# CompVis/behavior-driven-video-synthesis

Hardware: AMD Instinct MI355X
Metric: frames/sec VUnet 256x256 bs=16 fwd+bwd (higher is better)
Workload: dtype f32 (operands scaled by a power of two and split into 2 fp16 terms, 3 partial products on fp16 MFMA, fp32 accumulate; weight gradients and uncovered layers: 3 bf16 terms / 6 products, fp32-input MFMA, fp32 VALU); 1 GPU; Human3.6m shape_and_pose_net VunetAlter 256x256 per-GPU bs=16 fwd+bwd, VGG19 perceptual + KL loss, fused Adam, dropout 0.05, regressor side loop off, seeded-synthetic VGG19 weights, rasterised synthetic stickmen; global_batch=16, parallelism=dp1, conv_precision=h2, hip_streams=4, hip_graph=True, graph_settle_steps=7, rccl_world_size=1, dp_backend=none

## Files before the change

### behavior_driven_video_synthesis_amd/csrc/planes.hip

```cpp
#include "common.h"
#include "split_h2.h"

namespace {

constexpr int P2_AMAX0 = 16, P2_NSLOT = 64;

__device__ __forceinline__ void p2_unpack8(const uint4& h, const uint4& l, float inv, float* v) {
  const uint32_t hs[4] = {h.x, h.y, h.z, h.w}, ls[4] = {l.x, l.y, l.z, l.w};
#pragma unroll
  for (int j = 0; j < 4; ++j) {
    const h2_f16x2 a = __builtin_bit_cast(h2_f16x2, hs[j]), b = __builtin_bit_cast(h2_f16x2, ls[j]);
    v[2 * j] = ((float)a[0] + (float)b[0] * (1.f / 2048.f)) * inv;
    v[2 * j + 1] = ((float)a[1] + (float)b[1] * (1.f / 2048.f)) * inv;
  }
}
__device__ __forceinline__ void p2_pack8(const float* v, float s, uint4& h, uint4& l) {
  h2_split2(v[0] * s, v[1] * s, h.x, l.x);
  h2_split2(v[2] * s, v[3] * s, h.y, l.y);
  h2_split2(v[4] * s, v[5] * s, h.z, l.z);
  h2_split2(v[6] * s, v[7] * s, h.w, l.w);
}
__device__ __forceinline__ float block_sum4(float v, float* red) {
  v = wave_sum(v);
  __syncthreads();
  if ((threadIdx.x & 63) == 0) red[threadIdx.x >> 6] = v;
  __syncthreads();
  return red[0] + red[1] + red[2] + red[3];
}
__device__ __forceinline__ float meta_amax(const int* meta) {
  return wave_max(__int_as_float(meta[P2_AMAX0 + (threadIdx.x & (P2_NSLOT - 1))]));
}
__device__ __forceinline__ void publish_amax(int* meta, float vmax) {
  const float m = wave_max(vmax);
  if ((threadIdx.x & 63) == 0)
    atomicMax(reinterpret_cast<unsigned*>(meta) + P2_AMAX0 + ((blockIdx.x * 4u + (threadIdx.x >> 6)) & (P2_NSLOT - 1)), __float_as_uint(m));
}

__global__ __launch_bounds__(256) void p2_finish_sum_kernel(const float* partial, int nb, float* out, float scale) {
  __shared__ float red[4];
  float s = 0.f;
  for (int i = threadIdx.x; i < nb; i += 256) s += partial[i];
  const float t = block_sum4(s, red);
  if (threadIdx.x == 0) out[0] += scale * t;
}

__global__ __launch_bounds__(256) void p2_l1_partial_kernel(const uint4* __restrict__ t, const int* __restrict__ tmeta,
                                                            const uint4* __restrict__ p, const int* __restrict__ pmeta,
                                                            float* __restrict__ partial, size_t plane) {
  __shared__ float red[4];
  const float it = h2_pow2(-tmeta[0]), ip = h2_pow2(-pmeta[0]);
  float s = 0.f;
  for (size_t i = (size_t)blockIdx.x * 256 + threadIdx.x; i < plane; i += (size_t)gridDim.x * 256) {
    float a[8], b[8];
    p2_unpack8(t[i], t[plane + i], it, a);
    p2_unpack8(p[i], p[plane + i], ip, b);
    s += ((fabsf(a[0] - b[0]) + fabsf(a[1] - b[1])) + (fabsf(a[2] - b[2]) + fabsf(a[3] - b[3]))) +
         ((fabsf(a[4] - b[4]) + fabsf(a[5] - b[5])) + (fabsf(a[6] - b[6]) + fabsf(a[7] - b[7])));
  }
  const float tot = block_sum4(s, red);
  if (threadIdx.x == 0) partial[blockIdx.x] = tot;
}

template <bool L1>
__global__ __launch_bounds__(256) void p2_pool_fwd_kernel(const uint4* __restrict__ t, const int* __restrict__ tmeta,
                                                          const uint4* __restrict__ p, const int* __restrict__ pmeta,
                                                          float* __restrict__ partial, uint4* __restrict__ y, int* __restrict__ ymeta,
                                                          int NCB, int H, int W) {
  __shared__ float red[4];
  const int Ho = H >> 1, Wo = W >> 1, Wp = W + 2, Wpo = Wo + 2;
  const size_t plane = (size_t)NCB * (H + 2) * Wp, plane_o = (size_t)NCB * (Ho + 2) * Wpo, total = (size_t)NCB * Ho * Wo;
  const float ip = h2_pow2(-pmeta[0]);
  const float it = L1 ? h2_pow2(-tmeta[0]) : 0.f;
  if (blockIdx.x == 0 && threadIdx.x < 64) {
    if (threadIdx.x == 0) ymeta[0] = pmeta[0];
    ymeta[P2_AMAX0 + threadIdx.x] = pmeta[P2_AMAX0 + threadIdx.x];
  }
  float s = 0.f;
  for (size_t o = (size_t)blockIdx.x * 256 + threadIdx.x; o < total; o += (size_t)gridDim.x * 256) {
    const int xo = (int)(o % Wo);
    size_t r = o / Wo;
    const int yo = (int)(r % Ho);
    const size_t ncb = r / Ho;
    const size_t i0 = (ncb * (H + 2) + (2 * yo + 1)) * Wp + (2 * xo + 1);
    const size_t off[4] = {i0, i0 + 1, i0 + Wp, i0 + Wp + 1};
    uint32_t hs[4][4], ls[4][4];
    float v[4][8];
#pragma unroll
    for (int e = 0; e < 4; ++e) {
      const uint4 h = p[off[e]], l = p[plane + off[e]];
      hs[e][0] = h.x; hs[e][1] = h.y; hs[e][2] = h.z; hs[e][3] = h.w;
      ls[e][0] = l.x; ls[e][1] = l.y; ls[e][2] = l.z; ls[e][3] = l.w;
      p2_unpack8(h, l, ip, v[e]);
    }
    if (L1) {
#pragma unroll
      for (int e = 0; e < 4; ++e) {
        float a[8];
        p2_unpack8(t[off[e]], t[plane + off[e]], it, a);
#pragma unroll
        for (int j = 0; j < 8; ++j) s += fabsf(a[j] - v[e][j]);
      }
    }
    uint32_t oh[4] = {0, 0, 0, 0}, ol[4] = {0, 0, 0, 0};
#pragma unroll
    for (int j = 0; j < 8; ++j) {
      const float m = fmaxf(fmaxf(v[0][j], v[1][j]), fmaxf(v[2][j], v[3][j]));
      const int k = v[0][j] == m ? 0 : (v[1][j] == m ? 1 : (v[2][j] == m ? 2 : 3));
      const uint32_t hsel = k == 0 ? hs[0][j >> 1] : (k == 1 ? hs[1][j >> 1] : (k == 2 ? hs[2][j >> 1] : hs[3][j >> 1]));
      const uint32_t lsel = k == 0 ? ls[0][j >> 1] : (k == 1 ? ls[1][j >> 1] : (k == 2 ? ls[2][j >> 1] : ls[3][j >> 1]));
      const uint32_t keep = (j & 1) ? 0xFFFF0000u : 0x0000FFFFu;
      oh[j >> 1] |= hsel & keep;
      ol[j >> 1] |= lsel & keep;
    }
    const size_t oo = (ncb * (Ho + 2) + (yo + 1)) * Wpo + (xo + 1);
    y[oo] = make_uint4(oh[0], oh[1], oh[2], oh[3]);
    y[plane_o + oo] = make_uint4(ol[0], ol[1], ol[2], ol[3]);
  }
  if (L1) {
    const float tot = block_sum4(s, red);
    if (threadIdx.x == 0) partial[blockIdx.x] = tot;
  }
}

__global__ __launch_bounds__(256) void p2_l1_bwd_kernel(const uint4* __restrict__ t, const int* __restrict__ tmeta,
                                                        const uint4* __restrict__ p, const int* __restrict__ pmeta,
                                                        const uint4* __restrict__ add, const int* __restrict__ addmeta,
                                                        uint4* __restrict__ g, int* __restrict__ gmeta, float gscale,
                                                        const float* __restrict__ gout, int NCB, int H, int W) {
  const float c = gscale * (gout ? gout[0] : 1.f);
  const float bound = (add ? meta_amax(addmeta) : 0.f) + fabsf(c);
  const int eg = h2_scale_exp(bound);
  const float sg = h2_pow2(eg);
  if (blockIdx.x == 0 && threadIdx.x == 0) gmeta[0] = eg;
  const float it = h2_pow2(-tmeta[0]), ip = h2_pow2(-pmeta[0]), ia = add ? h2_pow2(-addmeta[0]) : 0.f;
  const int Wp = W + 2;
  const size_t plane = (size_t)NCB * (H + 2) * Wp, total = (size_t)NCB * H * W;
  float vmax = 0.f;
  for (size_t o = (size_t)blockIdx.x * 256 + threadIdx.x; o < total; o += (size_t)gridDim.x * 256) {
    const int xw = (int)(o % W);
    size_t r = o / W;
    const int yh = (int)(r % H);
    const size_t i = ((r / H) * (H + 2) + (yh + 1)) * Wp + (xw + 1);
    float a[8], b[8], d[8];
    p2_unpack8(t[i], t[plane + i], it, a);
    p2_unpack8(p[i], p[plane + i], ip, b);
    if (add) p2_unpack8(add[i], add[plane + i], ia, d);
#pragma unroll
    for (int j = 0; j < 8; ++j) {
      const float df = b[j] - a[j];
      float v = (add ? d[j] : 0.f) + (df > 0.f ? c : (df < 0.f ? -c : 0.f));
      if (!(b[j] > 0.f)) v = 0.f;
      d[j] = v;
      vmax = fmaxf(vmax, fabsf(v));
    }
    uint4 h, l;
    p2_pack8(d, sg, h, l);
    g[i] = h;
    g[plane + i] = l;
  }
  publish_amax(gmeta, vmax);
}

template <bool L1>
__global__ __launch_bounds__(256) void p2_pool_bwd_kernel(const uint4* __restrict__ t, const int* __restrict__ tmeta,
                                                          const uint4* __restrict__ p, const int* __restrict__ pmeta,
                                                          const uint4* __restrict__ dy, const int* __restrict__ dymeta,
                                                          uint4* __restrict__ g, int* __restrict__ gmeta, float gscale,
                                                          const float* __restrict__ gout, int NCB, int H, int W) {
  const float c = L1 ? gscale * (gout ? gout[0] : 1.f) : 0.f;
  const float bound = meta_amax(dymeta) + fabsf(c);
  const int eg = h2_scale_exp(bound);
  const float sg = h2_pow2(eg);
  if (blockIdx.x == 0 && threadIdx.x == 0) gmeta[0] = eg;
  const float ip = h2_pow2(-pmeta[0]), idy = h2_pow2(-dymeta[0]);
  const float it = L1 ? h2_pow2(-tmeta[0]) : 0.f;
  const int Ho = H >> 1, Wo = W >> 1, Wp = W + 2, Wpo = Wo + 2;
  const size_t plane = (size_t)NCB * (H + 2) * Wp, plane_o = (size_t)NCB * (Ho + 2) * Wpo, total = (size_t)NCB * Ho * Wo;
  float vmax = 0.f;
  for (size_t o = (size_t)blockIdx.x * 256 + threadIdx.x; o < total; o += (size_t)gridDim.x * 256) {
    const int xo = (int)(o % Wo);
    size_t r = o / Wo;
    const int yo = (int)(r % Ho);
    const size_t ncb = r / Ho;
    const size_t i0 = (ncb * (H + 2) + (2 * yo + 1)) * Wp + (2 * xo + 1);
    const size_t off[4] = {i0, i0 + 1, i0 + Wp, i0 + Wp + 1};
    const size_t oo = (ncb * (Ho + 2) + (yo + 1)) * Wpo + (xo + 1);
    float v[4][8], gy[8];
#pragma unroll
    for (int e = 0; e < 4; ++e) p2_unpack8(p[off[e]], p[plane + off[e]], ip, v[e]);
    p2_unpack8(dy[oo], dy[plane_o + oo], idy, gy);
    float res[4][8];
#pragma unroll
    for (int j = 0; j < 8; ++j) {
      const float m = fmaxf(fmaxf(v[0][j], v[1][j]), fmaxf(v[2][j], v[3][j]));
      const int k = v[0][j] == m ? 0 : (v[1][j] == m ? 1 : (v[2][j] == m ? 2 : 3));
#pragma unroll
      for (int e = 0; e < 4; ++e) res[e][j] = k == e ? gy[j] : 0.f;
    }
#pragma unroll
    for (int e = 0; e < 4; ++e) {
      float a[8];
      if (L1) p2_unpack8(t[off[e]], t[plane + off[e]], it, a);
#pragma unroll
      for (int j = 0; j < 8; ++j) {
        float x = res[e][j];
        if (L1) {
          const float df = v[e][j] - a[j];
          x += df > 0.f ? c : (df < 0.f ? -c : 0.f);
        }
        if (!(v[e][j] > 0.f)) x = 0.f;
        res[e][j] = x;
        vmax = fmaxf(vmax, fabsf(x));
      }
      uint4 h, l;
      p2_pack8(res[e], sg, h, l);
      g[off[e]] = h;
      g[plane + off[e]] = l;
    }
  }
  publish_amax(gmeta, vmax);
}

inline unsigned grid_for(size_t n, unsigned cap) {
  size_t b = (n + 255) / 256;
  if (b > cap) b = cap;
  if (b < 1) b = 1;
  return (unsigned)b;
}

}

extern "C" int vunet_p2_l1_fwd(const void* t, const int32_t* tmeta, const void* p, const int32_t* pmeta, float* partial, float* out,
                               float weight, int32_t N, int32_t C, int32_t H, int32_t W, void* stream) {
  if (!t || !tmeta || !p || !pmeta || !partial || !out || C % 8 || N < 1) return VUNET_ERR_ARG;
  const size_t plane = (size_t)N * (C / 8) * (H + 2) * (W + 2);
  const unsigned nb = grid_for(plane, 1024);
  hipStream_t st = (hipStream_t)stream;
  VUNET_LAUNCH(p2_l1_partial_kernel, dim3(nb), dim3(256), 0, st, (const uint4*)t, (const int*)tmeta, (const uint4*)p, (const int*)pmeta,
               partial, plane);
  VUNET_LAUNCH(p2_finish_sum_kernel, dim3(1), dim3(256), 0, st, (const float*)partial, (int)nb, out,
               weight / ((float)N * C * H * W));
  return vunet_check_launch();
}

extern "C" int vunet_p2_pool_fwd(const void* t, const int32_t* tmeta, const void* p, const int32_t* pmeta, float* partial, float* out,
                                 float weight, void* y, int32_t* ymeta, int32_t N, int32_t C, int32_t H, int32_t W, void* stream) {
  if (!p || !pmeta || !y || !ymeta || C % 8 || N < 1 || (H & 1) || (W & 1)) return VUNET_ERR_ARG;
  if (t && (!tmeta || !partial || !out)) return VUNET_ERR_ARG;
  const int NCB = N * (C / 8);
  const size_t total = (size_t)NCB * (H / 2) * (W / 2);
  const unsigned nb = grid_for(total, 1024);
  hipStream_t st = (hipStream_t)stream;
  if (t) {
    VUNET_LAUNCH(p2_pool_fwd_kernel<true>, dim3(nb), dim3(256), 0, st, (const uint4*)t, (const int*)tmeta, (const uint4*)p,
                 (const int*)pmeta, partial, (uint4*)y, (int*)ymeta, NCB, (int)H, (int)W);
    VUNET_LAUNCH(p2_finish_sum_kernel, dim3(1), dim3(256), 0, st, (const float*)partial, (int)nb, out,
                 weight / ((float)N * C * H * W));
  } else {
    VUNET_LAUNCH(p2_pool_fwd_kernel<false>, dim3(nb), dim3(256), 0, st, (const uint4*)nullptr, (const int*)nullptr, (const uint4*)p,
                 (const int*)pmeta, (float*)nullptr, (uint4*)y, (int*)ymeta, NCB, (int)H, (int)W);
  }
  return vunet_check_launch();
}

extern "C" int vunet_p2_l1_bwd(const void* t, const int32_t* tmeta, const void* p, const int32_t* pmeta, const void* add,
                               const int32_t* addmeta, void* g, int32_t* gmeta, float gscale, const float* gout, int32_t N, int32_t C,
                               int32_t H, int32_t W, void* stream) {
  if (!t || !tmeta || !p || !pmeta || !g || !gmeta || C % 8 || N < 1 || (add && !addmeta)) return VUNET_ERR_ARG;
  const int NCB = N * (C / 8);
  const size_t total = (size_t)NCB * H * W;
  VUNET_LAUNCH(p2_l1_bwd_kernel, dim3(grid_for(total, 2048)), dim3(256), 0, (hipStream_t)stream, (const uint4*)t, (const int*)tmeta,
               (const uint4*)p, (const int*)pmeta, (const uint4*)add, (const int*)addmeta, (uint4*)g, (int*)gmeta, gscale, gout, NCB,
               (int)H, (int)W);
  return vunet_check_launch();
}

extern "C" int vunet_p2_pool_bwd(const void* t, const int32_t* tmeta, const void* p, const int32_t* pmeta, const void* dy,
                                 const int32_t* dymeta, void* g, int32_t* gmeta, float gscale, const float* gout, int32_t N, int32_t C,
                                 int32_t H, int32_t W, void* stream) {
  if (!p || !pmeta || !dy || !dymeta || !g || !gmeta || C % 8 || N < 1 || (H & 1) || (W & 1) || (t && !tmeta)) return VUNET_ERR_ARG;
  const int NCB = N * (C / 8);
  const size_t total = (size_t)NCB * (H / 2) * (W / 2);
  const unsigned nb = grid_for(total, 2048);
  hipStream_t st = (hipStream_t)stream;
  if (t)
    VUNET_LAUNCH(p2_pool_bwd_kernel<true>, dim3(nb), dim3(256), 0, st, (const uint4*)t, (const int*)tmeta, (const uint4*)p,
                 (const int*)pmeta, (const uint4*)dy, (const int*)dymeta, (uint4*)g, (int*)gmeta, gscale, gout, NCB, (int)H, (int)W);
  else
    VUNET_LAUNCH(p2_pool_bwd_kernel<false>, dim3(nb), dim3(256), 0, st, (const uint4*)nullptr, (const int*)nullptr, (const uint4*)p,
                 (const int*)pmeta, (const uint4*)dy, (const int*)dymeta, (uint4*)g, (int*)gmeta, 0.f, (const float*)nullptr, NCB, (int)H,
                 (int)W);
  return vunet_check_launch();
}
```

### behavior_driven_video_synthesis_amd/models/imagenet_pretrained.py

```python
from __future__ import annotations

import math

import torch
from torch import nn

from .. import ops
from ..lib.modules import Conv2d

VGG19_CFG = [64, 64, "M", 128, 128, "M", 256, 256, 256, 256, "M", 512, 512, 512, 512, "M", 512, 512, 512, 512, "M"]


class _Marker(nn.Module):

    def __init__(self, kind):
        super().__init__()
        self.kind = kind


class VGG19(nn.Module):

    def __init__(self, width_div: int = 1):
        super().__init__()
        layers, cin = [], 3
# ... 118 lines not shown
                break
            if isinstance(m, Conv2d):
                nxt = mods[i + 1] if i + 1 < len(mods) else None
                if nxt is None or not (isinstance(nxt[1], _Marker) and nxt[1].kind == "relu"):
                    return None
                tap = taps.get(nxt[0])
                if first is None:
                    if tap is not None:
                        return None
                    first = m
                else:
                    steps.append(("conv", m, tap))
                i += 2
            elif isinstance(m, _Marker) and m.kind == "pool":
                if first is None:
                    return None
                steps.append(("pool",))
                i += 1
            else:
                return None
        if first is None or not steps or steps[-1][0] != "conv" or steps[-1][2] is None:
            return None
        return first, steps

    def shapes(self):
        first, steps = self.program
        n, h, w = self.geo
        c = first.weight.shape[0]
        out = [(c, h, w)]
        for st in steps:
            if st[0] == "pool":
                if h % 2 or w % 2:
                    return None
                h, w = h // 2, w // 2
            else:
                m = st[1]
                if m.weight.shape[1] != c or tuple(m.weight.shape[2:]) != (3, 3) or not ops.p2_conv_supported(n, c, h, w, m.weight.shape[0]):
                    return None
                if not ops.p2_conv_supported(n, m.weight.shape[0], h, w, c):
                    return None
                c = m.weight.shape[0]
            out.append((c, h, w))
        return out

    def _role(self, role):
        st = self.roles.get(role)
        if st is None:
            shp = self.shapes()
            n = self.geo[0]
            L = len(shp)
            metas = torch.zeros(3 * L, ops.P2_META_INTS, device=self.device, dtype=torch.int32)
            acts = [ops.Planes((n, c, h, w), self.device, meta=metas[k]) for k, (c, h, w) in enumerate(shp)]
            st = self.roles[role] = {"metas": metas, "A": acts, "G": [None] * L, "U": [None] * L, "shp": shp}
        return st

    def _grad_buf(self, st, kind, k):
        lst = st[kind]
        if lst[k] is None:
            c, h, w = st["shp"][k]
            L = len(st["shp"])
            lst[k] = ops.Planes((self.geo[0], c, h, w), self.device, meta=st["metas"][(1 if kind == "G" else 2) * L + k])
        return lst[k]

    @staticmethod
    def _weights(m):
        w = m.__dict__.get("_p2w")
        if w is None or w.weight is not m.weight:
            w = ops.P2Weights(m.weight, m.bias)
            object.__setattr__(m, "_p2w", w)
        return w

    def _first(self):
        m = self.program[0]
        stamp = (m.weight.data_ptr(), m.weight._version, m.bias._version)
        rec = m.__dict__.get("_p2first")
        if rec is None or rec[0] != stamp:
            w, b = m.weight.detach().contiguous(), m.bias.detach().contiguous()
            wt_f, wt_d, _, shift, _, _, wx_d = ops.pack_weights(w, None, b, None, None, 3, 0, 1, True)
            wk = torch.empty(4, device=w.device, dtype=torch.float32)
            work = torch.empty(2 * w.shape[0], device=w.device, dtype=torch.float32)
            ops._call("vunet_p2_weight_bound", ops._p(w), ops._p(b), int(w.shape[0]), 3, ops._p(wk), ops._p(work), ops._stream())
            rec = (stamp, wt_f, wt_d, shift, wx_d, wk)
            object.__setattr__(m, "_p2first", rec)
        return rec

    def forward(self, role, xp, targets=None, tap_weights=None):
        st = self._role(role)
        st["metas"].zero_()
        A = st["A"]
        _, wt_f, _, shift, _, wk = self._first()
        n, _, h, w = xp.shape
        amax = ops._tagged_amax(xp)
        if amax is None:
            amax = ops.absmax_partials(xp)
        ops._call("vunet_p2_conv_first", ops._p(xp), ops._p(amax), 512, ops._p(wt_f), int(wt_f.shape[1]), ops._p(shift), ops._p(wk),
                  ops._p(A[0].buf), ops._p(A[0].meta), n, h, w, A[0].shape[1], ops._stream())
        taps, losses = {}, {}
        steps = self.program[1]
        for k, step in enumerate(steps, start=1):
            if step[0] == "conv":
                ops.p2_conv(A[k - 1], self._weights(step[1]), A[k], relu=True)
                tap = step[2]
                if tap is not None:
                    taps[tap] = A[k]
                    pool_next = k < len(steps) and steps[k][0] == "pool"
                    if targets is not None and not pool_next:
                        losses[tap] = ops.p2_l1_fwd(targets[tap], A[k], tap_weights[tap])
            else:
                prev = steps[k - 2] if k >= 2 else None
                tap = prev[2] if (prev is not None and prev[0] == "conv") else None
                if targets is not None and tap is not None:
                    losses[tap] = ops.p2_pool_fwd(A[k - 1], A[k], t=targets[tap], weight=tap_weights[tap])
                else:
                    ops.p2_pool_fwd(A[k - 1], A[k])
        return taps, losses

    def backward(self, targets, tap_weights, gouts):
        st = self.roles["p"]
        A, steps = st["A"], self.program[1]
        L = len(steps)

        def tap_scale(tap, k):
            c, h, w = st["shp"][k]
            return float(tap_weights[tap]) / (self.geo[0] * c * h * w)

        def has(tap):
            return tap is not None and gouts.get(tap) is not None
        k = L
        top = steps[L - 1][2]
        D = None
        if has(top):
            D = ops.p2_l1_bwd(targets[top], A[L], None, self._grad_buf(st, "G", L), tap_scale(top, L), gouts[top])
        while k >= 1:
            step = steps[k - 1]
            if step[0] == "pool":
                prev = steps[k - 2]
                tap = prev[2] if has(prev[2]) else None
                if D is None and tap is None:
                    k -= 1
                    continue
                if D is None:
                    D = ops.p2_l1_bwd(targets[tap], A[k - 1], None, self._grad_buf(st, "G", k - 1), tap_scale(tap, k - 1), gouts[tap])
                else:
                    D = ops.p2_pool_bwd(A[k - 1], D, self._grad_buf(st, "G", k - 1), t=None if tap is None else targets[tap],
                                        gscale=0.0 if tap is None else tap_scale(tap, k - 1), gout=None if tap is None else gouts[tap])
                k -= 1
                continue
            below = steps[k - 2] if k >= 2 else None
            if D is None:
                tap = below[2] if (below is not None and below[0] == "conv" and has(below[2])) else None
                if tap is not None:
                    D = ops.p2_l1_bwd(targets[tap], A[k - 1], None, self._grad_buf(st, "G", k - 1), tap_scale(tap, k - 1), gouts[tap])
                k -= 1
                continue
            wts = self._weights(step[1])
            if below is None:
                D = ops.p2_conv(D, wts, self._grad_buf(st, "G", 0), dgrad=True, mask=A[0])
            elif below[0] == "pool":
                D = ops.p2_conv(D, wts, self._grad_buf(st, "G", k - 1), dgrad=True)
            elif has(below[2]):
                up = ops.p2_conv(D, wts, self._grad_buf(st, "U", k - 1), dgrad=True)
                D = ops.p2_l1_bwd(targets[below[2]], A[k - 1], up, self._grad_buf(st, "G", k - 1), tap_scale(below[2], k - 1),
                                  gouts[below[2]])
            else:
                D = ops.p2_conv(D, wts, self._grad_buf(st, "G", k - 1), dgrad=True, mask=A[k - 1])
            k -= 1
        if D is None:
            return None
        _, _, wt_d, _, wx_d, _ = self._first()
        n, h, w = self.geo
        c0 = st["shp"][0][0]
        dconv = D.to_nchw()
        dx = torch.empty(n, 3, h, w, device=self.device, dtype=torch.float32)
        ops._conv_gather(ops._dgrad_desc(n, c0, h, w, 3, h, w, 3, 1, 1, wt_d.shape[1]), dconv, None, wt_d, None, None, None, dx, wx_d)
        return dx


class P2VggLoss(torch.autograd.Function):

    @staticmethod
    def forward(ctx, xp, engine, target, tap_weights, names):
        _, losses = engine.forward("p", xp, target.planes, tap_weights)
        engine.pred_generation += 1
        ctx.engine, ctx.target, ctx.tap_weights, ctx.names = engine, target, tap_weights, names
        ctx.generation, ctx.pred_generation = target.generation, engine.pred_generation
        return tuple(losses[n] for n in names)

    @staticmethod
    def backward(ctx, *gouts):
        if ctx.target.generation != ctx.generation:
            raise RuntimeError("P2VggLoss.backward: the target features were overwritten by a later target pass of the same "
                               "PerceptualVGG (its planes buffers are persistent): run forward + backward per target")
        if ctx.engine.pred_generation != ctx.pred_generation:
            raise RuntimeError("P2VggLoss.backward: a later vgg_loss() of the same PerceptualVGG and input geometry has overwritten "
                               "this pass's activations (persistent planes buffers): call backward() before the next vgg_loss(), "
                               "or switch the planes path off (models.imagenet_pretrained.enable_p2(False)) for this use")
        g = ctx.engine.backward(ctx.target.planes, ctx.tap_weights,
                                {n: (None if go is None else go.contiguous()) for n, go in zip(ctx.names, gouts)})
        return g, None, None, None, None


class PerceptualVGG(nn.Module):

    def __init__(self, vgg, weights):
        super().__init__()
        feats = vgg.module.features if isinstance(vgg, nn.DataParallel) else vgg.features
        self.vgg_layers = _adopt_features(feats)
        self.loss_weights = weights
        self.register_buffer("mean", torch.tensor([0.485, 0.456, 0.406], dtype=torch.float).view(1, 3, 1, 1))
        self.register_buffer("std", torch.tensor([0.229, 0.224, 0.225], dtype=torch.float).view(1, 3, 1, 1))
        self.target_layers = {"3": "relu1_2", "8": "relu2_2", "13": "relu3_2", "22": "relu4_2", "31": "relu5_2"}
        for p in self.vgg_layers.parameters():
            p.requires_grad_(False)

    def _walk(self, x, on_tap, on_tap_pool=None):
        x = on_tap("input", ops.VggPreprocess.apply(x))
# ... 100 lines not shown
```

### behavior_driven_video_synthesis_amd/ops.py

```python
from __future__ import annotations

import contextlib
import ctypes
import os
from collections import namedtuple
from dataclasses import dataclass
from typing import Optional, Tuple

import torch

from . import _lib

ACT_NONE, ACT_ELU, ACT_RELU, ACT_SIGMOID, ACT_LRELU = 0, 1, 2, 3, 4
SEED2_OFFSET = 0x9E3779B9


class ConvDesc(ctypes.Structure):
    _fields_ = [("N", ctypes.c_int32), ("C1", ctypes.c_int32), ("C2", ctypes.c_int32), ("Hs", ctypes.c_int32),
                ("Ws", ctypes.c_int32), ("M", ctypes.c_int32), ("m_off", ctypes.c_int32), ("Mpad", ctypes.c_int32),
                ("Ho", ctypes.c_int32), ("Wo", ctypes.c_int32), ("KH", ctypes.c_int32), ("KW", ctypes.c_int32),
                ("stride", ctypes.c_int32), ("pad", ctypes.c_int32), ("mode", ctypes.c_int32),
                ("in_act", ctypes.c_int32), ("in_slope", ctypes.c_float), ("drop_p", ctypes.c_float),
                ("drop_seed", ctypes.c_uint32), ("out_act", ctypes.c_int32), ("d2s", ctypes.c_int32),
                ("aux_act", ctypes.c_int32), ("aux_slope", ctypes.c_float), ("aux_drop_p", ctypes.c_float),
# ... 1728 lines not shown


def _p2_key(d, dgrad):
    return (("conv_gather_dgrad" if dgrad else "conv_gather_fwd", d.N, d.C, 0, d.H, d.W, d.M, 3, 1, 0,
             _kernel_name("vunet_p2_conv_variant", ctypes.byref(d))), 2.0 * d.N * d.H * d.W * d.C * d.M * 9)


def p2_conv(x: Planes, wts: P2Weights, out: Planes, relu: bool = True, dgrad: bool = False, mask: Planes = None):
    n, c, h, w = x.shape
    m = wts.cin if dgrad else wts.cout
    assert c == (wts.cout if dgrad else wts.cin) and out.shape == (n, m, h, w)
    img, wk = wts.image(dgrad)
    d = P2Desc(n, c, h, w, m, int(relu and not dgrad))
    with _timed(_p2_key, d, dgrad):
        _call("vunet_p2_conv", ctypes.byref(d), _p(x.buf), _p(x.meta), _p(img), _p(wk),
              _p(None if dgrad or wts.bias is None else wts.bias), _p(None if mask is None else mask.buf), _p(out.buf), _p(out.meta),
              _stream())
    return out


def p2_l1_fwd(t: Planes, p: Planes, weight: float):
    n, c, h, w = p.shape
    assert t.shape == p.shape
    out = _zero_scalar(p.buf.device)
    partial = torch.empty(1024, device=p.buf.device, dtype=torch.float32)
    _call("vunet_p2_l1_fwd", _p(t.buf), _p(t.meta), _p(p.buf), _p(p.meta), _p(partial), _p(out), float(weight), n, c, h, w, _stream())
    return out


def p2_pool_fwd(p: Planes, out: Planes, t: Planes = None, weight: float = 0.0):
    n, c, h, w = p.shape
    assert out.shape == (n, c, h // 2, w // 2)
    loss = partial = None
    if t is not None:
        loss = _zero_scalar(p.buf.device)
        partial = torch.empty(1024, device=p.buf.device, dtype=torch.float32)
    _call("vunet_p2_pool_fwd", _p(None if t is None else t.buf), _p(None if t is None else t.meta), _p(p.buf), _p(p.meta), _p(partial),
          _p(loss), float(weight), _p(out.buf), _p(out.meta), n, c, h, w, _stream())
    return loss


def p2_l1_bwd(t: Planes, p: Planes, add, g: Planes, gscale: float, gout):
    n, c, h, w = p.shape
    _call("vunet_p2_l1_bwd", _p(t.buf), _p(t.meta), _p(p.buf), _p(p.meta), _p(None if add is None else add.buf),
          _p(None if add is None else add.meta), _p(g.buf), _p(g.meta), float(gscale), _p(gout), n, c, h, w, _stream())
    return g


def p2_pool_bwd(p: Planes, dy: Planes, g: Planes, t: Planes = None, gscale: float = 0.0, gout=None):
    n, c, h, w = p.shape
    _call("vunet_p2_pool_bwd", _p(None if t is None else t.buf), _p(None if t is None else t.meta), _p(p.buf), _p(p.meta), _p(dy.buf),
          _p(dy.meta), _p(g.buf), _p(g.meta), float(gscale), _p(gout), n, c, h, w, _stream())
    return g
```

### include/vunet_hip.h

```cpp
#ifndef VUNET_HIP_H
#define VUNET_HIP_H
#include <stddef.h>
#include <stdint.h>

#ifdef __cplusplus
extern "C" {
#endif

#define VUNET_OK 0
#define VUNET_ERR_ARG (-1)
#define VUNET_ERR_LAUNCH (-2)
#define VUNET_ERR_UNSUPPORTED (-3)

#define VUNET_ACT_NONE 0
#define VUNET_ACT_ELU 1
#define VUNET_ACT_RELU 2
#define VUNET_ACT_SIGMOID 3
#define VUNET_ACT_LRELU 4

int vunet_abi_version(void);

typedef struct vunet_conv_desc {
  int32_t N;
  int32_t C1, C2;
// ... 217 lines not shown
int vunet_dp_unique_id(void* id128);
int vunet_dp_init(int32_t world, int32_t rank, const void* id128);
int vunet_dp_world(void);
int vunet_dp_allreduce_bucket(float* buf, int64_t n, int32_t average, void* stream);
int vunet_dp_finalize(void);

int vunet_crop_window(const float* x, float* y, int32_t planes, int32_t H, int32_t W, int32_t P, const int32_t* off,
                      void* stream);
int vunet_crop_window_bwd(const float* dy, float* dx, int32_t planes, int32_t H, int32_t W, int32_t P, const int32_t* off,
                          void* stream);

#define VUNET_LOSS_MAX_TERMS 8
int vunet_total_loss(const float* const* terms, int32_t n, const float* kl, const float* gamma, float gamma_const,
                     float ll_weight, int32_t use_kl, float* loss, float* ll, void* stream);
int vunet_total_loss_bwd(const float* g_loss, const float* g_ll, int32_t n, const float* gamma, float gamma_const,
                         float ll_weight, int32_t use_kl, float* d, void* stream);
int vunet_gamma_update(float* gamma, const float* imax, const float* avg_kl, float gamma_step, void* stream);

int vunet_unit_sample(const float* mu, const float* logstd, float* z, float* eps_out, int64_t n, uint32_t seed, void* stream);

int vunet_set_schedule(double* lr_dev, double lr, float* imax_dev, float imax, int32_t* step_dev, int32_t step, void* stream);

int vunet_sum_amax(const float* const* srcs, int32_t n, float* out, float* amax_out, int64_t numel, void* stream);

typedef struct vunet_p2_desc {
  int32_t N, C, H, W;
  int32_t M;
  int32_t relu;
} vunet_p2_desc;
int vunet_p2_conv_supported(const vunet_p2_desc* d);
int vunet_p2_conv_variant(const vunet_p2_desc* d, char* name, int32_t len);
int vunet_p2_conv(const vunet_p2_desc* d, const void* x, const int32_t* xmeta, const void* w_image, const float* wk,
                  const float* shift, const void* mask, void* y, int32_t* ymeta, void* stream);
int vunet_p2_weight_image_bytes(int32_t Cout, int32_t Cin, int32_t dgrad);
int vunet_p2_pack_weights(const float* w, const float* shift, int32_t Cout, int32_t Cin, int32_t dgrad, void* image, float* wk,
                          float* workspace, void* stream);
int vunet_p2_weight_bound(const float* w, const float* shift, int32_t Cout, int32_t Cin, float* wk, float* workspace, void* stream);
int vunet_p2_conv_first(const float* x, const float* amax_x, int32_t n_amax, const float* wt_f, int32_t Mpad, const float* shift,
                        const float* wk, void* y, int32_t* ymeta, int32_t N, int32_t H, int32_t W, int32_t M, void* stream);
int vunet_p2_from_nchw(const float* x, const float* amax, int32_t n_amax, int32_t relu, void* y, int32_t* ymeta, int32_t N,
                       int32_t C, int32_t H, int32_t W, void* stream);
int vunet_p2_to_nchw(const void* x, const int32_t* xmeta, float* y, int32_t N, int32_t C, int32_t H, int32_t W, void* stream);

int vunet_p2_l1_fwd(const void* t, const int32_t* tmeta, const void* p, const int32_t* pmeta, float* partial, float* out,
                    float weight, int32_t N, int32_t C, int32_t H, int32_t W, void* stream);
int vunet_p2_pool_fwd(const void* t, const int32_t* tmeta, const void* p, const int32_t* pmeta, float* partial, float* out,
                      float weight, void* y, int32_t* ymeta, int32_t N, int32_t C, int32_t H, int32_t W, void* stream);
int vunet_p2_l1_bwd(const void* t, const int32_t* tmeta, const void* p, const int32_t* pmeta, const void* add,
                    const int32_t* addmeta, void* g, int32_t* gmeta, float gscale, const float* gout, int32_t N, int32_t C,
                    int32_t H, int32_t W, void* stream);
int vunet_p2_pool_bwd(const void* t, const int32_t* tmeta, const void* p, const int32_t* pmeta, const void* dy,
                      const int32_t* dymeta, void* g, int32_t* gmeta, float gscale, const float* gout, int32_t N, int32_t C,
                      int32_t H, int32_t W, void* stream);

typedef struct vunet_seq_linear_desc {
  int32_t B, M, K, ldx, act0, act1, nets, shared_in, S;
} vunet_seq_linear_desc;
typedef struct vunet_seq_coupling_desc {
  int32_t B, C, c1, ld_in, ld_out, Mp, reverse, affine_on_src, S;
} vunet_seq_coupling_desc;
typedef struct vunet_seq_lstm_desc {
  int32_t B, H, ldx, hoff, n, ldraw;
  int64_t seq_stride;
} vunet_seq_lstm_desc;
int vunet_seq_linear(const vunet_seq_linear_desc* d, const float* w0, const float* w1, const float* x, const float* bias0,
                     const float* bias1, float* y, void* stream);
int vunet_seq_coupling(const vunet_seq_coupling_desc* d, const float* in, const float* st, const float* bias_s, const float* bias_t,
                       const int32_t* map, const float* scale, const float* loc, float* out, float* logdet, void* stream);
int vunet_seq_start(const float* x0, int64_t x0_stride, const float* h0, const float* c0, float* xraw, int32_t ldraw, float* xh,
                    int32_t ldx, int32_t hoff, float* c, int32_t B, int32_t n, int32_t H, void* stream);
int vunet_seq_lstm_gates(const vunet_seq_lstm_desc* d, const float* w_perm, const float* xh, const float* bias_perm, const float* c_in,
                         float* c_out, float* xh_next, float* h_out, const float* x_next, void* stream);
int vunet_seq_decoder_out(const vunet_seq_lstm_desc* d, float* xh, const float* w_out, const float* b_out, float* xraw, float* xs,
                          float* cs, void* stream);
int vunet_seq_lstm_bias(const float* b_ih, const float* b_hh, const float* fold, int32_t H, float* bias_perm, void* stream);
int vunet_seq_fold_input(const float* w_ih, const float* w_in, const float* b_in, int32_t M, int32_t n, float* w_fold,
                         float* bias_fold, void* stream);
int vunet_seq_bottleneck(const float* heads, int32_t Mp, const float* eps, float* mu, float* logstd, float* b_out, int32_t B,
                         int32_t H, void* stream);
int vunet_seq_pack_rows(const float* src, int32_t M, int32_t K, const float* row_scale, float* dst, int32_t ld_dst, int32_t col_off,
                        int32_t row_off, int32_t row_mul, void* stream);
int vunet_seq_pose_project(const float* x, int32_t n_use, const int32_t* dims_to_use, const double* mean, const double* stdv, int32_t D,
                           int32_t f32_math, const double* cam, float* kps, int32_t T, int32_t J, void* stream);
int vunet_seq_actnorm_init(const float* x, int32_t ld, int32_t B, int32_t C, float* loc, float* scale, void* stream);
int vunet_seq_normlinear_rows(const float* v, const float* g, const float* bias, const float* gamma, const float* beta, int32_t M,
                              int32_t K, float* row_scale, float* bias_eff, void* stream);

int vunet_seq_slerp(const float* b1, const float* b2, int64_t ld_in, int pairs, int h, const double* steps, int n_steps, float* out,
                    void* stream);

#ifdef __cplusplus
}
#endif
#endif
```

Baseline: 808.9 frames/s.

## Store compact 2-bit sign/argmax codes in VGG forward to slim backward passes

During the perceptual-loss VGG forward, the L1 and pool kernels now also write packed 2-bit state codes: ReLU-active plus the sign of prediction minus target, and the max-pool argmax index. The backward L1 and pool kernels read these codes instead of reloading the full two-plane fp16 activations and targets. This cuts backward memory traffic and recomputation, at the cost of extra code writes in the forward pass and extra code buffers. It is on by default through an environment flag.

```diff
diff --git a/behavior_driven_video_synthesis_amd/csrc/planes.hip b/behavior_driven_video_synthesis_amd/csrc/planes.hip
--- a/behavior_driven_video_synthesis_amd/csrc/planes.hip
+++ b/behavior_driven_video_synthesis_amd/csrc/planes.hip
@@ -19,6 +19,10 @@
   h2_split2(v[2] * s, v[3] * s, h.y, l.y);
   h2_split2(v[4] * s, v[5] * s, h.z, l.z);
   h2_split2(v[6] * s, v[7] * s, h.w, l.w);
+}
+__device__ __forceinline__ uint32_t p2_state(float p, float t) {
+  const float df = p - t;
+  return !(p > 0.f) ? 0u : (df > 0.f ? 1u : (df < 0.f ? 2u : 3u));
 }
 __device__ __forceinline__ float block_sum4(float v, float* red) {
   v = wave_sum(v);
@@ -44,9 +48,10 @@
   if (threadIdx.x == 0) out[0] += scale * t;
 }
 
+template <bool CODE>
 __global__ __launch_bounds__(256) void p2_l1_partial_kernel(const uint4* __restrict__ t, const int* __restrict__ tmeta,
                                                             const uint4* __restrict__ p, const int* __restrict__ pmeta,
-                                                            float* __restrict__ partial, size_t plane) {
+                                                            float* __restrict__ partial, uint16_t* __restrict__ code, size_t plane) {
   __shared__ float red[4];
   const float it = h2_pow2(-tmeta[0]), ip = h2_pow2(-pmeta[0]);
   float s = 0.f;
@@ -56,16 +61,22 @@
     p2_unpack8(p[i], p[plane + i], ip, b);
     s += ((fabsf(a[0] - b[0]) + fabsf(a[1] - b[1])) + (fabsf(a[2] - b[2]) + fabsf(a[3] - b[3]))) +
          ((fabsf(a[4] - b[4]) + fabsf(a[5] - b[5])) + (fabsf(a[6] - b[6]) + fabsf(a[7] - b[7])));
+    if (CODE) {
+      uint32_t cw = 0;
+#pragma unroll
+      for (int j = 0; j < 8; ++j) cw |= p2_state(b[j], a[j]) << (2 * j);
+      code[i] = (uint16_t)cw;
+    }
   }
   const float tot = block_sum4(s, red);
   if (threadIdx.x == 0) partial[blockIdx.x] = tot;
 }
 
-template <bool L1>
+template <bool L1, bool CODE>
 __global__ __launch_bounds__(256) void p2_pool_fwd_kernel(const uint4* __restrict__ t, const int* __restrict__ tmeta,
                                                           const uint4* __restrict__ p, const int* __restrict__ pmeta,
                                                           float* __restrict__ partial, uint4* __restrict__ y, int* __restrict__ ymeta,
-                                                          int NCB, int H, int W) {
+                                                          uint4* __restrict__ code, int NCB, int H, int W) {
   __shared__ float red[4];
   const int Ho = H >> 1, Wo = W >> 1, Wp = W + 2, Wpo = Wo + 2;
   const size_t plane = (size_t)NCB * (H + 2) * Wp, plane_o = (size_t)NCB * (Ho + 2) * Wpo, total = (size_t)NCB * Ho * Wo;
@@ -92,20 +103,30 @@
       ls[e][0] = l.x; ls[e][1] = l.y; ls[e][2] = l.z; ls[e][3] = l.w;
       p2_unpack8(h, l, ip, v[e]);
     }
+    uint32_t ck = 0, cs[4] = {0, 0, 0, 0};
     if (L1) {
 #pragma unroll
       for (int e = 0; e < 4; ++e) {
         float a[8];
         p2_unpack8(t[off[e]], t[plane + off[e]], it, a);
 #pragma unroll
-        for (int j = 0; j < 8; ++j) s += fabsf(a[j] - v[e][j]);
+        for (int j = 0; j < 8; ++j) {
+          s += fabsf(a[j] - v[e][j]);
+          if (CODE) cs[e] |= p2_state(v[e][j], a[j]) << (2 * j);
+        }
       }
+    } else if (CODE) {
+#pragma unroll
+      for (int e = 0; e < 4; ++e)
+#pragma unroll
+        for (int j = 0; j < 8; ++j) cs[e] |= (v[e][j] > 0.f ? 3u : 0u) << (2 * j);
     }
     uint32_t oh[4] = {0, 0, 0, 0}, ol[4] = {0, 0, 0, 0};
 #pragma unroll
     for (int j = 0; j < 8; ++j) {
       const float m = fmaxf(fmaxf(v[0][j], v[1][j]), fmaxf(v[2][j], v[3][j]));
       const int k = v[0][j] == m ? 0 : (v[1][j] == m ? 1 : (v[2][j] == m ? 2 : 3));
+      if (CODE) ck |= (uint32_t)k << (2 * j);
       const uint32_t hsel = k == 0 ? hs[0][j >> 1] : (k == 1 ? hs[1][j >> 1] : (k == 2 ? hs[2][j >> 1] : hs[3][j >> 1]));
       const uint32_t lsel = k == 0 ? ls[0][j >> 1] : (k == 1 ? ls[1][j >> 1] : (k == 2 ? ls[2][j >> 1] : ls[3][j >> 1]));
       const uint32_t keep = (j & 1) ? 0xFFFF0000u : 0x0000FFFFu;
@@ -115,6 +136,7 @@
     const size_t oo = (ncb * (Ho + 2) + (yo + 1)) * Wpo + (xo + 1);
     y[oo] = make_uint4(oh[0], oh[1], oh[2], oh[3]);
     y[plane_o + oo] = make_uint4(ol[0], ol[1], ol[2], ol[3]);
+    if (CODE) code[o] = make_uint4(ck, cs[0] | (cs[1] << 16), cs[2] | (cs[3] << 16), 0u);
   }
   if (L1) {
     const float tot = block_sum4(s, red);
@@ -221,6 +243,91 @@
   publish_amax(gmeta, vmax);
 }
 
+__global__ __launch_bounds__(256) void p2_l1_bwd_code_kernel(const uint16_t* __restrict__ code, const uint4* __restrict__ add,
+                                                             const int* __restrict__ addmeta, uint4* __restrict__ g,
+                                                             int* __restrict__ gmeta, float gscale, const float* __restrict__ gout,
+                                                             int NCB, int H, int W) {
+  const float c = gscale * (gout ? gout[0] : 1.f);
+  const float bound = (add ? meta_amax(addmeta) : 0.f) + fabsf(c);
+  const int eg = h2_scale_exp(bound);
+  const float sg = h2_pow2(eg);
+  if (blockIdx.x == 0 && threadIdx.x == 0) gmeta[0] = eg;
+  const float ia = add ? h2_pow2(-addmeta[0]) : 0.f;
+  const int Wp = W + 2;
+  const size_t plane = (size_t)NCB * (H + 2) * Wp, total = (size_t)NCB * H * W;
+  float vmax = 0.f;
+  for (size_t o = (size_t)blockIdx.x * 256 + threadIdx.x; o < total; o += (size_t)gridDim.x * 256) {
+    const int xw = (int)(o % W);
+    size_t r = o / W;
+    const int yh = (int)(r % H);
+    const size_t i = ((r / H) * (H + 2) + (yh + 1)) * Wp + (xw + 1);
+    const uint32_t cw = code[i];
+    float d[8];
+    if (add) p2_unpack8(add[i], add[plane + i], ia, d);
+#pragma unroll
+    for (int j = 0; j < 8; ++j) {
+      const uint32_t st = (cw >> (2 * j)) & 3u;
+      float v = (add ? d[j] : 0.f) + (st == 1u ? c : (st == 2u ? -c : 0.f));
+      if (st == 0u) v = 0.f;
+      d[j] = v;
+      vmax = fmaxf(vmax, fabsf(v));
+    }
+    uint4 h, l;
+    p2_pack8(d, sg, h, l);
+    g[i] = h;
+    g[plane + i] = l;
+  }
+  publish_amax(gmeta, vmax);
+}
+
+template <bool L1>
+__global__ __launch_bounds__(256) void p2_pool_bwd_code_kernel(const uint4* __restrict__ code, const uint4* __restrict__ dy,
+                                                               const int* __restrict__ dymeta, uint4* __restrict__ g,
+                                                               int* __restrict__ gmeta, float gscale, const float* __restrict__ gout,
+                                                               int NCB, int H, int W) {
+  const float c = L1 ? gscale * (gout ? gout[0] : 1.f) : 0.f;
+  const float bound = meta_amax(dymeta) + fabsf(c);
+  const int eg = h2_scale_exp(bound);
+  const float sg = h2_pow2(eg);
+  if (blockIdx.x == 0 && threadIdx.x == 0) gmeta[0] = eg;
+  const float idy = h2_pow2(-dymeta[0]);
+  const int Ho = H >> 1, Wo = W >> 1, Wp = W + 2, Wpo = Wo + 2;
+  const size_t plane = (size_t)NCB * (H + 2) * Wp, plane_o = (size_t)NCB * (Ho + 2) * Wpo, total = (size_t)NCB * Ho * Wo;
+  float vmax = 0.f;
+  for (size_t o = (size_t)blockIdx.x * 256 + threadIdx.x; o < total; o += (size_t)gridDim.x * 256) {
+    const int xo = (int)(o % Wo);
+    size_t r = o / Wo;
+    const int yo = (int)(r % Ho);
+    const size_t ncb = r / Ho;
+    const size_t i0 = (ncb * (H + 2) + (2 * yo + 1)) * Wp + (2 * xo + 1);
+    const size_t off[4] = {i0, i0 + 1, i0 + Wp, i0 + Wp + 1};
+    const size_t oo = (ncb * (Ho + 2) + (yo + 1)) * Wpo + (xo + 1);
+    const uint4 cw = code[o];
+    const uint32_t cs[4] = {cw.y & 0xFFFFu, cw.y >> 16, cw.z & 0xFFFFu, cw.z >> 16};
+    float gy[8];
+    p2_unpack8(dy[oo], dy[plane_o + oo], idy, gy);
+#pragma unroll
+    for (int e = 0; e < 4; ++e) {
+      float res[8];
+#pragma unroll
+      for (int j = 0; j < 8; ++j) {
+        const int k = (int)((cw.x >> (2 * j)) & 3u);
+        const uint32_t st = (cs[e] >> (2 * j)) & 3u;
+        float x = k == e ? gy[j] : 0.f;
+        if (L1) x += st == 1u ? c : (st == 2u ? -c : 0.f);
+        if (st == 0u) x = 0.f;
+        res[j] = x;
+        vmax = fmaxf(vmax, fabsf(x));
+      }
+      uint4 h, l;
+      p2_pack8(res, sg, h, l);
+      g[off[e]] = h;
+      g[plane + off[e]] = l;
+    }
+  }
+  publish_amax(gmeta, vmax);
+}
+
 inline unsigned grid_for(size_t n, unsigned cap) {
   size_t b = (n + 255) / 256;
   if (b > cap) b = cap;
@@ -230,37 +337,56 @@
 
 }
 
-extern "C" int vunet_p2_l1_fwd(const void* t, const int32_t* tmeta, const void* p, const int32_t* pmeta, float* partial, float* out,
-                               float weight, int32_t N, int32_t C, int32_t H, int32_t W, void* stream) {
+extern "C" int vunet_p2_l1_fwd_code(const void* t, const int32_t* tmeta, const void* p, const int32_t* pmeta, float* partial,
+                                    float* out, float weight, void* code, int32_t N, int32_t C, int32_t H, int32_t W, void* stream) {
   if (!t || !tmeta || !p || !pmeta || !partial || !out || C % 8 || N < 1) return VUNET_ERR_ARG;
   const size_t plane = (size_t)N * (C / 8) * (H + 2) * (W + 2);
   const unsigned nb = grid_for(plane, 1024);
   hipStream_t st = (hipStream_t)stream;
-  VUNET_LAUNCH(p2_l1_partial_kernel, dim3(nb), dim3(256), 0, st, (const uint4*)t, (const int*)tmeta, (const uint4*)p, (const int*)pmeta,
-               partial, plane);
+  if (code)
+    VUNET_LAUNCH(p2_l1_partial_kernel<true>, dim3(nb), dim3(256), 0, st, (const uint4*)t, (const int*)tmeta, (const uint4*)p,
+                 (const int*)pmeta, partial, (uint16_t*)code, plane);
+  else
+    VUNET_LAUNCH(p2_l1_partial_kernel<false>, dim3(nb), dim3(256), 0, st, (const uint4*)t, (const int*)tmeta, (const uint4*)p,
+                 (const int*)pmeta, partial, (uint16_t*)nullptr, plane);
   VUNET_LAUNCH(p2_finish_sum_kernel, dim3(1), dim3(256), 0, st, (const float*)partial, (int)nb, out,
                weight / ((float)N * C * H * W));
   return vunet_check_launch();
 }
 
-extern "C" int vunet_p2_pool_fwd(const void* t, const int32_t* tmeta, const void* p, const int32_t* pmeta, float* partial, float* out,
-                                 float weight, void* y, int32_t* ymeta, int32_t N, int32_t C, int32_t H, int32_t W, void* stream) {
+extern "C" int vunet_p2_l1_fwd(const void* t, const int32_t* tmeta, const void* p, const int32_t* pmeta, float* partial, float* out,
+                               float weight, int32_t N, int32_t C, int32_t H, int32_t W, void* stream) {
+  return vunet_p2_l1_fwd_code(t, tmeta, p, pmeta, partial, out, weight, nullptr, N, C, H, W, stream);
+}
+
+extern "C" int vunet_p2_pool_fwd_code(const void* t, const int32_t* tmeta, const void* p, const int32_t* pmeta, float* partial,
+                                      float* out, float weight, void* y, int32_t* ymeta, void* code, int32_t N, int32_t C, int32_t H,
+                                      int32_t W, void* stream) {
   if (!p || !pmeta || !y || !ymeta || C % 8 || N < 1 || (H & 1) || (W & 1)) return VUNET_ERR_ARG;
   if (t && (!tmeta || !partial || !out)) return VUNET_ERR_ARG;
   const int NCB = N * (C / 8);
   const size_t total = (size_t)NCB * (H / 2) * (W / 2);
   const unsigned nb = grid_for(total, 1024);
   hipStream_t st = (hipStream_t)stream;
+#define P2_POOL_FWD(L1, CODE, T, TM, PART)                                                                                  \
+  VUNET_LAUNCH((p2_pool_fwd_kernel<L1, CODE>), dim3(nb), dim3(256), 0, st, (const uint4*)(T), (const int*)(TM), (const uint4*)p, \
+               (const int*)pmeta, (float*)(PART), (uint4*)y, (int*)ymeta, (uint4*)code, NCB, (int)H, (int)W)
   if (t) {
-    VUNET_LAUNCH(p2_pool_fwd_kernel<true>, dim3(nb), dim3(256), 0, st, (const uint4*)t, (const int*)tmeta, (const uint4*)p,
-                 (const int*)pmeta, partial, (uint4*)y, (int*)ymeta, NCB, (int)H, (int)W);
+    if (code) P2_POOL_FWD(true, true, t, tmeta, partial);
+    else P2_POOL_FWD(true, false, t, tmeta, partial);
     VUNET_LAUNCH(p2_finish_sum_kernel, dim3(1), dim3(256), 0, st, (const float*)partial, (int)nb, out,
                  weight / ((float)N * C * H * W));
   } else {
-    VUNET_LAUNCH(p2_pool_fwd_kernel<false>, dim3(nb), dim3(256), 0, st, (const uint4*)nullptr, (const int*)nullptr, (const uint4*)p,
-                 (const int*)pmeta, (float*)nullptr, (uint4*)y, (int*)ymeta, NCB, (int)H, (int)W);
-  }
-  return vunet_check_launch();
+    if (code) P2_POOL_FWD(false, true, nullptr, nullptr, nullptr);
+    else P2_POOL_FWD(false, false, nullptr, nullptr, nullptr);
+  }
+#undef P2_POOL_FWD
+  return vunet_check_launch();
+}
+
+extern "C" int vunet_p2_pool_fwd(const void* t, const int32_t* tmeta, const void* p, const int32_t* pmeta, float* partial, float* out,
+                                 float weight, void* y, int32_t* ymeta, int32_t N, int32_t C, int32_t H, int32_t W, void* stream) {
+  return vunet_p2_pool_fwd_code(t, tmeta, p, pmeta, partial, out, weight, y, ymeta, nullptr, N, C, H, W, stream);
 }
 
 extern "C" int vunet_p2_l1_bwd(const void* t, const int32_t* tmeta, const void* p, const int32_t* pmeta, const void* add,
@@ -292,3 +418,29 @@
                  (int)W);
   return vunet_check_launch();
 }
+
+extern "C" int vunet_p2_l1_bwd_code(const void* code, const void* add, const int32_t* addmeta, void* g, int32_t* gmeta, float gscale,
+                                    const float* gout, int32_t N, int32_t C, int32_t H, int32_t W, void* stream) {
+  if (!code || !g || !gmeta || C % 8 || N < 1 || (add && !addmeta)) return VUNET_ERR_ARG;
+  const int NCB = N * (C / 8);
+  const size_t total = (size_t)NCB * H * W;
+  VUNET_LAUNCH(p2_l1_bwd_code_kernel, dim3(grid_for(total, 2048)), dim3(256), 0, (hipStream_t)stream, (const uint16_t*)code,
+               (const uint4*)add, (const int*)addmeta, (uint4*)g, (int*)gmeta, gscale, gout, NCB, (int)H, (int)W);
+  return vunet_check_launch();
+}
+
+extern "C" int vunet_p2_pool_bwd_code(const void* code, int32_t tap, const void* dy, const int32_t* dymeta, void* g, int32_t* gmeta,
+                                      float gscale, const float* gout, int32_t N, int32_t C, int32_t H, int32_t W, void* stream) {
+  if (!code || !dy || !dymeta || !g || !gmeta || C % 8 || N < 1 || (H & 1) || (W & 1)) return VUNET_ERR_ARG;
+  const int NCB = N * (C / 8);
+  const size_t total = (size_t)NCB * (H / 2) * (W / 2);
+  const unsigned nb = grid_for(total, 2048);
+  hipStream_t st = (hipStream_t)stream;
+  if (tap)
+    VUNET_LAUNCH(p2_pool_bwd_code_kernel<true>, dim3(nb), dim3(256), 0, st, (const uint4*)code, (const uint4*)dy, (const int*)dymeta,
+                 (uint4*)g, (int*)gmeta, gscale, gout, NCB, (int)H, (int)W);
+  else
+    VUNET_LAUNCH(p2_pool_bwd_code_kernel<false>, dim3(nb), dim3(256), 0, st, (const uint4*)code, (const uint4*)dy, (const int*)dymeta,
+                 (uint4*)g, (int*)gmeta, 0.f, (const float*)nullptr, NCB, (int)H, (int)W);
+  return vunet_check_launch();
+}
diff --git a/behavior_driven_video_synthesis_amd/models/imagenet_pretrained.py b/behavior_driven_video_synthesis_amd/models/imagenet_pretrained.py
--- a/behavior_driven_video_synthesis_amd/models/imagenet_pretrained.py
+++ b/behavior_driven_video_synthesis_amd/models/imagenet_pretrained.py
@@ -194,6 +194,15 @@
             metas = torch.zeros(3 * L, ops.P2_META_INTS, device=self.device, dtype=torch.int32)
             acts = [ops.Planes((n, c, h, w), self.device, meta=metas[k]) for k, (c, h, w) in enumerate(shp)]
             st = self.roles[role] = {"metas": metas, "A": acts, "G": [None] * L, "U": [None] * L, "shp": shp}
+            if role == "p":
+                steps = self.program[1]
+                codes = {}
+                for k, step in enumerate(steps, start=1):
+                    if step[0] == "pool":
+                        codes[k - 1] = ops.p2_pool_code(acts[k - 1])
+                    elif step[2] is not None and not (k < len(steps) and steps[k][0] == "pool"):
+                        codes[k] = ops.p2_l1_code(acts[k])
+                st["codes"], st["coded"] = codes, False
         return st
 
     def _grad_buf(self, st, kind, k):
@@ -239,6 +248,9 @@
                   ops._p(A[0].buf), ops._p(A[0].meta), n, h, w, A[0].shape[1], ops._stream())
         taps, losses = {}, {}
         steps = self.program[1]
+        codes = st["codes"] if (role == "p" and ops.p2_tap_codes["on"]) else None
+        if role == "p":
+            st["coded"] = codes is not None
         for k, step in enumerate(steps, start=1):
             if step[0] == "conv":
                 ops.p2_conv(A[k - 1], self._weights(step[1]), A[k], relu=True)
@@ -247,20 +259,29 @@
                     taps[tap] = A[k]
                     pool_next = k < len(steps) and steps[k][0] == "pool"
                     if targets is not None and not pool_next:
-                        losses[tap] = ops.p2_l1_fwd(targets[tap], A[k], tap_weights[tap])
+                        if codes is not None:
+                            losses[tap] = ops.p2_l1_fwd_code(targets[tap], A[k], tap_weights[tap], codes[k])
+                        else:
+                            losses[tap] = ops.p2_l1_fwd(targets[tap], A[k], tap_weights[tap])
             else:
                 prev = steps[k - 2] if k >= 2 else None
                 tap = prev[2] if (prev is not None and prev[0] == "conv") else None
-                if targets is not None and tap is not None:
-                    losses[tap] = ops.p2_pool_fwd(A[k - 1], A[k], t=targets[tap], weight=tap_weights[tap])
+                with_t = targets is not None and tap is not None
+                if codes is not None:
+                    loss = ops.p2_pool_fwd_code(A[k - 1], A[k], codes[k - 1], t=targets[tap] if with_t else None,
+                                                weight=tap_weights[tap] if with_t else 0.0)
                 else:
-                    ops.p2_pool_fwd(A[k - 1], A[k])
+                    loss = ops.p2_pool_fwd(A[k - 1], A[k], t=targets[tap] if with_t else None,
+                                           weight=tap_weights[tap] if with_t else 0.0)
+                if with_t:
+                    losses[tap] = loss
         return taps, losses
 
     def backward(self, targets, tap_weights, gouts):
         st = self.roles["p"]
         A, steps = st["A"], self.program[1]
         L = len(steps)
+        codes = st["codes"] if st["coded"] else None
 
         def tap_scale(tap, k):
             c, h, w = st["shp"][k]
@@ -268,11 +289,17 @@
 
         def has(tap):
             return tap is not None and gouts.get(tap) is not None
+
+        def l1_bwd(tap, k, add):
+            g = self._grad_buf(st, "G", k)
+            if codes is not None and not (k < L and steps[k][0] == "pool"):
+                return ops.p2_l1_bwd_code(codes[k], add, g, tap_scale(tap, k), gouts[tap])
+            return ops.p2_l1_bwd(targets[tap], A[k], add, g, tap_scale(tap, k), gouts[tap])
         k = L
         top = steps[L - 1][2]
         D = None
         if has(top):
-            D = ops.p2_l1_bwd(targets[top], A[L], None, self._grad_buf(st, "G", L), tap_scale(top, L), gouts[top])
+            D = l1_bwd(top, L, None)
         while k >= 1:
             step = steps[k - 1]
             if step[0] == "pool":
@@ -282,7 +309,11 @@
                     k -= 1
                     continue
                 if D is None:
-                    D = ops.p2_l1_bwd(targets[tap], A[k - 1], None, self._grad_buf(st, "G", k - 1), tap_scale(tap, k - 1), gouts[tap])
+                    D = l1_bwd(tap, k - 1, None)
+                elif codes is not None:
+                    D = ops.p2_pool_bwd_code(codes[k - 1], D, self._grad_buf(st, "G", k - 1), tap=tap is not None,
+                                             gscale=0.0 if tap is None else tap_scale(tap, k - 1),
+                                             gout=None if tap is None else gouts[tap])
                 else:
                     D = ops.p2_pool_bwd(A[k - 1], D, self._grad_buf(st, "G", k - 1), t=None if tap is None else targets[tap],
                                         gscale=0.0 if tap is None else tap_scale(tap, k - 1), gout=None if tap is None else gouts[tap])
@@ -292,7 +323,7 @@
             if D is None:
                 tap = below[2] if (below is not None and below[0] == "conv" and has(below[2])) else None
                 if tap is not None:
-                    D = ops.p2_l1_bwd(targets[tap], A[k - 1], None, self._grad_buf(st, "G", k - 1), tap_scale(tap, k - 1), gouts[tap])
+                    D = l1_bwd(tap, k - 1, None)
                 k -= 1
                 continue
             wts = self._weights(step[1])
@@ -302,8 +333,7 @@
                 D = ops.p2_conv(D, wts, self._grad_buf(st, "G", k - 1), dgrad=True)
             elif has(below[2]):
                 up = ops.p2_conv(D, wts, self._grad_buf(st, "U", k - 1), dgrad=True)
-                D = ops.p2_l1_bwd(targets[below[2]], A[k - 1], up, self._grad_buf(st, "G", k - 1), tap_scale(below[2], k - 1),
-                                  gouts[below[2]])
+                D = l1_bwd(below[2], k - 1, up)
             else:
                 D = ops.p2_conv(D, wts, self._grad_buf(st, "G", k - 1), dgrad=True, mask=A[k - 1])
             k -= 1
diff --git a/behavior_driven_video_synthesis_amd/ops.py b/behavior_driven_video_synthesis_amd/ops.py
--- a/behavior_driven_video_synthesis_amd/ops.py
+++ b/behavior_driven_video_synthesis_amd/ops.py
@@ -1804,3 +1804,54 @@
     _call("vunet_p2_pool_bwd", _p(None if t is None else t.buf), _p(None if t is None else t.meta), _p(p.buf), _p(p.meta), _p(dy.buf),
           _p(dy.meta), _p(g.buf), _p(g.meta), float(gscale), _p(gout), n, c, h, w, _stream())
     return g
+
+
+p2_tap_codes = {"on": os.environ.get("VUNET_P2_TAP_CODES", "1") != "0"}
+
+
+def p2_l1_code(p: Planes) -> torch.Tensor:
+    return torch.zeros(p.buf[0].numel() // 8, device=p.buf.device, dtype=torch.int16)
+
+
+def p2_pool_code(p: Planes) -> torch.Tensor:
+    n, c, h, w = p.shape
+    return torch.zeros(n * (c // 8) * (h // 2) * (w // 2), 4, device=p.buf.device, dtype=torch.int32)
+
+
+def p2_l1_fwd_code(t: Planes, p: Planes, weight: float, code: torch.Tensor):
+    n, c, h, w = p.shape
+    assert t.shape == p.shape and code.dtype == torch.int16 and code.numel() == p.buf[0].numel() // 8
+    out = _zero_scalar(p.buf.device)
+    partial = torch.empty(1024, device=p.buf.device, dtype=torch.float32)
+    _call("vunet_p2_l1_fwd_code", _p(t.buf), _p(t.meta), _p(p.buf), _p(p.meta), _p(partial), _p(out), float(weight), _p(code),
+          n, c, h, w, _stream())
+    return out
+
+
+def p2_pool_fwd_code(p: Planes, out: Planes, code: torch.Tensor, t: Planes = None, weight: float = 0.0):
+    n, c, h, w = p.shape
+    assert out.shape == (n, c, h // 2, w // 2)
+    assert code.dtype == torch.int32 and code.numel() == n * (c // 8) * (h // 2) * (w // 2) * 4
+    loss = partial = None
+    if t is not None:
+        loss = _zero_scalar(p.buf.device)
+        partial = torch.empty(1024, device=p.buf.device, dtype=torch.float32)
+    _call("vunet_p2_pool_fwd_code", _p(None if t is None else t.buf), _p(None if t is None else t.meta), _p(p.buf), _p(p.meta),
+          _p(partial), _p(loss), float(weight), _p(out.buf), _p(out.meta), _p(code), n, c, h, w, _stream())
+    return loss
+
+
+def p2_l1_bwd_code(code: torch.Tensor, add, g: Planes, gscale: float, gout):
+    n, c, h, w = g.shape
+    assert code.dtype == torch.int16 and code.numel() == g.buf[0].numel() // 8
+    _call("vunet_p2_l1_bwd_code", _p(code), _p(None if add is None else add.buf), _p(None if add is None else add.meta), _p(g.buf),
+          _p(g.meta), float(gscale), _p(gout), n, c, h, w, _stream())
+    return g
+
+
+def p2_pool_bwd_code(code: torch.Tensor, dy: Planes, g: Planes, tap: bool = False, gscale: float = 0.0, gout=None):
+    n, c, h, w = g.shape
+    assert code.dtype == torch.int32 and code.numel() == n * (c // 8) * (h // 2) * (w // 2) * 4
+    _call("vunet_p2_pool_bwd_code", _p(code), int(bool(tap)), _p(dy.buf), _p(dy.meta), _p(g.buf), _p(g.meta), float(gscale), _p(gout),
+          n, c, h, w, _stream())
+    return g
diff --git a/include/vunet_hip.h b/include/vunet_hip.h
--- a/include/vunet_hip.h
+++ b/include/vunet_hip.h
@@ -293,6 +293,15 @@
 int vunet_p2_pool_bwd(const void* t, const int32_t* tmeta, const void* p, const int32_t* pmeta, const void* dy,
                       const int32_t* dymeta, void* g, int32_t* gmeta, float gscale, const float* gout, int32_t N, int32_t C,
                       int32_t H, int32_t W, void* stream);
+int vunet_p2_l1_fwd_code(const void* t, const int32_t* tmeta, const void* p, const int32_t* pmeta, float* partial, float* out,
+                         float weight, void* code, int32_t N, int32_t C, int32_t H, int32_t W, void* stream);
+int vunet_p2_pool_fwd_code(const void* t, const int32_t* tmeta, const void* p, const int32_t* pmeta, float* partial, float* out,
+                           float weight, void* y, int32_t* ymeta, void* code, int32_t N, int32_t C, int32_t H, int32_t W,
+                           void* stream);
+int vunet_p2_l1_bwd_code(const void* code, const void* add, const int32_t* addmeta, void* g, int32_t* gmeta, float gscale,
+                         const float* gout, int32_t N, int32_t C, int32_t H, int32_t W, void* stream);
+int vunet_p2_pool_bwd_code(const void* code, int32_t tap, const void* dy, const int32_t* dymeta, void* g, int32_t* gmeta,
+                           float gscale, const float* gout, int32_t N, int32_t C, int32_t H, int32_t W, void* stream);
 
 typedef struct vunet_seq_linear_desc {
   int32_t B, M, K, ldx, act0, act1, nets, shared_in, S;
```

Result: no change. 815.1 frames/s, median of 6 (+0.8%).
